# OChicken/GPQHE

Hardware: AMD Instinct MI355X
Metric: ciphertext he_mul/sec (RNS core: tensor 30 limbs + key-switch 45 limbs), N=2^16 (higher is better)
Workload: dtype u64; 1 GPU; he_mul RNS core, n=2^16, dimA=30, dimB=45, batch=64 ciphertexts per GPU (BASELINE configs[2]); he_rescale has no RNS-domain work in the reference; batch_per_gpu=64, total_batch=64, chunk=32, parallelism=ciphertext-per-GPU x1, no data-path collective, launcher=single process

## Files before the change

gpqhe_amd/_native.py:

```python
import ctypes as C
import os

_HERE = os.path.dirname(os.path.abspath(__file__))
LIB_PATH = os.path.join(_HERE, "libgpqhe_hip.so")


def use_variant(path):
    global LIB_PATH
    if _lib is not None:
        raise RuntimeError("use_variant(%r): the library is already loaded" % path)
    if not os.path.exists(path):
        raise FileNotFoundError(path)
    LIB_PATH = os.path.abspath(path)


u64 = C.c_uint64
vp = C.c_void_p

SIGNATURES = {
    "gpq_ctx_create": (C.c_int, [C.POINTER(vp), C.c_uint, C.c_uint, C.c_int]),
    "gpq_ctx_create_from_tables": (C.c_int, [C.POINTER(vp), C.c_uint, C.c_uint, C.POINTER(u64),
                                             C.POINTER(C.POINTER(u64)), C.POINTER(C.POINTER(u64)), C.c_int]),
    "gpq_ctx_destroy": (None, [vp]),
    "gpq_ctx_logn": (C.c_uint, [vp]),
# ... 28 lines not shown
    "gpq_mulpt_rns": (C.c_int, [vp] * 6 + [C.c_uint, C.c_uint, vp]),
    "gpq_set_chunk": (C.c_int, [vp, C.c_uint]),
    "gpq_set_limb_block": (C.c_int, [vp, C.c_uint]),
    "gpq_set_limb_classes": (C.c_int, [vp, C.c_uint, C.c_uint]),
    "gpq_tensor_workspace_bytes": (C.c_size_t, [vp, C.c_uint, C.c_uint]),
    "gpq_keyswitch_workspace_bytes": (C.c_size_t, [vp, C.c_uint, C.c_uint]),
    "gpq_he_mul_tensor": (C.c_int, [vp] * 8 + [C.c_uint, C.c_uint, vp, vp]),
    "gpq_keyswitch": (C.c_int, [vp] * 6 + [C.c_uint, C.c_uint, vp, vp]),
    "gpq_big_words": (C.c_uint, [C.c_uint]),
    "gpq_ctx_phat_invmp": (u64, [vp, C.c_uint, C.c_uint]),
    "gpq_ctx_pbits": (C.c_uint, [vp, C.c_uint]),
    "gpq_rns_decompose": (C.c_int, [vp, vp, vp, C.c_uint, C.c_uint, C.c_uint, vp]),
    "gpq_rns_decompose_limbs": (C.c_int, [vp, vp, vp, C.c_uint, C.c_uint, C.c_uint, C.c_uint, vp]),
    "gpq_rns_reconstruct": (C.c_int, [vp, vp, C.c_uint, vp, C.c_uint, C.c_uint, C.c_uint, vp]),
    "gpq_rns_reconstruct_one": (C.c_int, [vp, C.POINTER(u64), C.c_uint, C.POINTER(u64), C.c_uint]),
    "gpq_set_exact_crt": (C.c_int, [vp, C.c_int]),
    "gpq_set_stream_bridge": (C.c_int, [vp, C.c_int]),
    "gpq_debug_force_redo": (C.c_int, [vp, C.c_uint]),
    "gpq_debug_split_entry_fits_wide": (C.c_int, [u64, u64, u64]),
    "gpq_debug_zero_watch": (C.c_int, [vp, C.c_int]),
    "gpq_debug_zero_flags": (C.c_long, [vp, vp, vp, C.c_size_t]),
    "gpq_set_lazy_decompose": (C.c_int, [vp, C.c_int]),
    "gpq_set_nt_policy": (C.c_int, [vp, C.c_int]),
    "gpq_set_overlap": (C.c_int, [vp, C.c_int]),
    "gpq_last_lanes": (C.c_uint, [vp]),
    "gpq_debug_fail_peer": (C.c_int, [vp, C.c_int]),
    "gpq_debug_table_bytes": (C.c_size_t, [vp, C.c_int]),
    "gpq_set_fused_tail": (C.c_int, [vp, C.c_int]),
    "gpq_big_transpose": (C.c_int, [vp, vp, vp, C.c_uint, C.c_uint, C.c_int, vp]),
    "gpq_big_addsub": (C.c_int, [vp, vp, vp, vp, C.c_uint, C.c_uint, C.c_int, vp]),
    "gpq_set_prescale": (C.c_int, [vp, C.c_int]),
    "gpq_set_bridge_mfma": (C.c_int, [vp, C.c_int]),
    "gpq_poly_mul_workspace_bytes": (C.c_size_t, [vp, C.c_uint, C.c_uint]),
    "gpq_poly_mul": (C.c_int, [vp, vp, vp, vp, C.c_uint, C.c_uint, C.c_uint, C.c_uint, vp, vp]),
    "gpq_poly_mul_general_workspace_bytes": (C.c_size_t, [vp, C.c_uint, C.c_uint]),
    "gpq_rns_reconstruct_general": (C.c_int, [vp, vp, C.c_uint, vp, C.c_uint, C.c_uint, C.POINTER(u64), C.c_uint, vp, vp]),
    "gpq_poly_mul_general": (C.c_int, [vp, vp, vp, vp, C.c_uint, C.c_uint, C.POINTER(u64), C.c_uint, C.c_uint, vp, vp]),
    "gpq_he_rs": (C.c_int, [vp, vp, vp, C.c_uint, C.c_uint, C.c_uint, C.c_uint, vp]),
    "gpq_he_rescale": (C.c_int, [vp, vp, vp, C.c_uint, C.c_uint, C.c_uint, C.c_uint, vp]),
    "gpq_he_dims": (C.c_int, [vp, C.c_uint, C.c_uint] + [C.POINTER(C.c_uint)] * 4),
    "gpq_he_mul_workspace_bytes": (C.c_size_t, [vp, C.c_uint, C.c_uint, C.c_uint, C.c_uint, C.c_uint]),
    "gpq_he_mul": (C.c_int, [vp] * 9 + [C.c_uint] * 6 + [vp, vp]),
    "gpq_he_mul_rs": (C.c_int, [vp] * 9 + [C.c_uint] * 7 + [vp, vp]),
    "gpq_relin_tail_workspace_bytes": (C.c_size_t, [vp, C.c_uint, C.c_uint, C.c_uint, C.c_uint]),
    "gpq_relin_tail": (C.c_int, [vp, vp, vp, vp, C.c_uint, C.c_uint, C.c_uint, C.c_uint, C.c_uint, vp, vp]),
    "gpq_relin_tail_overwriting": (C.c_int, [vp, vp, vp, vp, C.c_uint, C.c_uint, C.c_uint, C.c_uint, C.c_uint, vp, vp]),
# ... 133 lines not shown
```

gpqhe_amd/csrc/engine.hip:

```cpp
#include "../../include/gpqhe_hip.h"
#include "engine_internal.hpp"
#include "ntt_kernels.hpp"

#include <cmath>
#include <cstdlib>
#include <cstdarg>
#include <cstdio>
#include <cstring>
#include <new>
#include <type_traits>

using namespace gpq;

static thread_local char g_err[512] = "";

int gpq_fail(int code, const char *fmt, ...) {
  va_list ap;
  va_start(ap, fmt);
  vsnprintf(g_err, sizeof g_err, fmt, ap);
  va_end(ap);
  return code;
}
extern "C" const char *gpq_last_error(void) { return g_err; }

// ... 417 lines not shown
template <typename TW_, int LOW_, bool NT_>
struct Mid8Inst { using TW = TW_; static constexpr int LOW = LOW_; static constexpr bool NT = NT_; };
template <typename F>
static int launch_mid8(const gpq_ctx *c, const PassArgs &m, unsigned limbs, const uint64_t **evk0, const uint64_t **evk1, int slot, hipStream_t s, F launch) {
  return for_limb_ranges<true>(c, m, limbs, evk0, evk1, [&](auto tag, const PassArgs &a, unsigned nl) {
    using TW = decltype(tag);
    ProfScope prof(c, slot, s);
    with_nt(a.nt, [&](auto nt) {
      constexpr bool NT = decltype(nt)::value;
      if (c->low9) launch(Mid8Inst<TW, 9, NT>{}, a, nl);
      else launch(Mid8Inst<TW, 8, NT>{}, a, nl);
    });
    return (int)GPQ_OK;
  });
}
template <typename K>
static int launch_mid8(const gpq_ctx *c, const PassArgs &m, unsigned limbs, unsigned polys, int slot, hipStream_t s, K kernel) {
  return launch_mid8(c, m, limbs, nullptr, nullptr, slot, s, [&](auto inst, const PassArgs &a, unsigned nl) {
    hipLaunchKernelGGL(kernel(inst), dim3(c->n >> 11, polys, nl), dim3(CONTIG_WAVES * 64), 0, s, a);
  });
}
template <typename K, typename... Tail>
static int launch_keyswitch_mid8(const gpq_ctx *c, KeyswitchArgs m, unsigned limbs, unsigned polys, int slot, hipStream_t s, K kernel, Tail... tail) {
  return launch_mid8(c, m.p, limbs, &m.evk0, &m.evk1, slot, s, [&](auto inst, const PassArgs &a, unsigned nl) {
    KeyswitchArgs ka{a, m.evk0, m.evk1};
    const dim3 block(CONTIG_WAVES * 64);
    if (polys / 2) hipLaunchKernelGGL(kernel(inst, std::true_type{}), dim3(c->n >> 11, polys / 2, nl), block, 0, s, ka, 0u, tail...);
    if (polys & 1) hipLaunchKernelGGL(kernel(inst, std::false_type{}), dim3(c->n >> 11, 1, nl), block, 0, s, ka, polys - 1, tail...);
  });
}

template <int M1, int EL, bool INV, bool CANON, typename TW, int CW = 8>
int launch_strided_t(const PassArgs &a, unsigned gy, unsigned gz, hipStream_t s) {
  using G = StridedGeom<M1, EL>;
  with_nt(a.nt, [&](auto nt) {
    hipLaunchKernelGGL((strided_pass<M1, EL, INV, CANON, TW, CW, decltype(nt)::value>), dim3((1u << CW) >> G::CB, gy, gz), dim3(G::T), 0, s, a);
  });
  return GPQ_OK;
}

template <bool INV>
int launch_strided(const gpq_ctx *c, const PassArgs &args, unsigned dim, unsigned polys, hipStream_t s) {
  return for_limb_ranges<true>(c, args, dim, nullptr, nullptr, [&](auto tag, const PassArgs &a, unsigned limbs) {
    using TW = decltype(tag);
    ProfScope prof(c, INV ? GPQ_K_STRIDED_INV : GPQ_K_STRIDED_FWD, s);
    switch (c->logn) {
      case 13: return launch_strided_t<5, 4, INV, false, TW>(a, polys * a.nslab, limbs, s);
      case 14: return launch_strided_t<6, 4, INV, false, TW>(a, polys * a.nslab, limbs, s);
// ... 314 lines not shown
      for (unsigned i = 0; i < nin; ++i) m.src[i] = f.dst[i];
      m.dst[0] = d0 + k0 * poly + loff; m.dst[1] = d1 + k0 * poly + loff; m.dst[2] = d2 + k0 * poly + loff;
      if ((rc = launch_mid8(c, m, limbs, polys, GPQ_K_TENSOR_MID, s, [&](auto i) {
            using I = decltype(i);
            return square ? tensor_sq_mid8<typename I::TW, I::LOW, I::NT> : tensor_mid8<typename I::TW, I::LOW, I::NT>;
          }))) return rc;
      PassArgs b = make_args(c, dim, 3, nt);
      b.limb0 = l0;
      if (inv_tabs) b.tabs = inv_tabs;
      for (int i = 0; i < 3; ++i) { b.src[i] = m.dst[i]; b.dst[i] = m.dst[i]; }
      if ((rc = launch_strided<true>(c, b, limbs, polys, s))) return rc;
    }
    return (int)GPQ_OK;
  };
  if ((rc = gpq_launch_groups(c, s, batch, chunk, gpq_lane_key(3, dim, chunk, 0, 0, 0), [&](gpq_ctx *q) { return inv_tabs ? 0 : gpq_tensor_workspace_bytes(q, dim, chunk); }, own, peer))) return rc;
  return after_launch("gpq_he_mul_tensor");
}

extern "C" int gpq_keyswitch(gpq_ctx *c, uint64_t *c0, uint64_t *c1, const uint64_t *x,
                             const uint64_t *evk0, const uint64_t *evk1,
                             unsigned dim, unsigned batch, void *workspace, void *stream) {
  return gpq_keyswitch_scaled(c, c0, c1, x, evk0, evk1, dim, batch, workspace, stream, nullptr);
}
int gpq_keyswitch_scaled(gpq_ctx *c, uint64_t *c0, uint64_t *c1, const uint64_t *x, const uint64_t *evk0, const uint64_t *evk1, unsigned dim,
                         unsigned batch, void *workspace, void *stream, const LimbTab *inv_tabs) {
  int rc = check_shape(c, dim, batch, "gpq_keyswitch");
  if (rc) return rc;
  if (!c0 || !c1 || !x || !evk0 || !evk1 || !workspace) return gpq_fail(GPQ_ERR_INVALID, "gpq_keyswitch: null pointer");
  hipStream_t s = (hipStream_t)stream;
  const size_t poly = (size_t)dim << c->logn;
  uint64_t *ws = (uint64_t *)workspace;

  if (!two_pass(c)) {
    HIP_TRY(hipMemcpyAsync(ws, x, batch * poly * 8, hipMemcpyDeviceToDevice, s));
    if ((rc = gpq_ntt(c, ws, dim, batch, stream))) return rc;
    for (unsigned k = 0; k < batch; ++k) {
      if ((rc = gpq_rns_mul(c, c0 + k * poly, ws + k * poly, evk0, dim, 1, stream))) return rc;
      if ((rc = gpq_rns_mul(c, c1 + k * poly, ws + k * poly, evk1, dim, 1, stream))) return rc;
    }
    if ((rc = gpq_invntt(c, c0, dim, batch, stream))) return rc;
    return gpq_invntt(c, c1, dim, batch, stream);
  }

  const unsigned chunk = gpq_group_size(c, batch);
  const unsigned lblock = limb_block(c, dim);
  auto peer = [&](const PeerLane &lane, unsigned k0, unsigned polys) {
    const size_t o = k0 * poly;
    return gpq_keyswitch_scaled(lane.c, c0 + o, c1 + o, x + o, evk0, evk1, dim, polys, lane.ws, lane.s, inv_tabs);
  };
  auto own = [&](unsigned k0, unsigned polys) {
    int rc;
    for (unsigned l0 = 0; l0 < dim; l0 += lblock) {
      const unsigned limbs = dim - l0 < lblock ? dim - l0 : lblock;
      const size_t loff = (size_t)l0 << c->logn;
      StageRange stage("gpq_keyswitch: strided fwd / keyswitch_mid8x2 / strided inv x2");
      const unsigned nt = nt_for(c, polys, limbs, 3);
      PassArgs f = make_args(c, dim, 1, nt);
      f.limb0 = l0;
      f.src[0] = x + k0 * poly + loff; f.dst[0] = ws + loff;
      if ((rc = launch_strided<false>(c, f, limbs, polys, s))) return rc;
      KeyswitchArgs m;
      m.p = make_args(c, dim, 1, nt);
      m.p.limb0 = l0;
      m.p.src[0] = f.dst[0]; m.p.dst[0] = c0 + k0 * poly + loff; m.p.dst[1] = c1 + k0 * poly + loff;
      m.evk0 = evk0 + loff; m.evk1 = evk1 + loff;
      if ((rc = launch_keyswitch_mid8(c, m, limbs, polys, GPQ_K_KEYSWITCH_MID, s, [](auto i, auto two) {
            using I = decltype(i);
            return keyswitch_mid8x2<typename I::TW, I::LOW, decltype(two)::value, I::NT>;
          }))) return rc;
      PassArgs b = make_args(c, dim, 2, nt);
      b.limb0 = l0;
      if (inv_tabs) b.tabs = inv_tabs;
      for (int i = 0; i < 2; ++i) { b.src[i] = m.p.dst[i]; b.dst[i] = m.p.dst[i]; }
      if ((rc = launch_strided<true>(c, b, limbs, polys, s))) return rc;
    }
    return (int)GPQ_OK;
  };
  if ((rc = gpq_launch_groups(c, s, batch, chunk, gpq_lane_key(4, dim, chunk, 0, 0, 0), [&](gpq_ctx *q) { return inv_tabs ? 0 : gpq_keyswitch_workspace_bytes(q, dim, chunk); }, own, peer))) return rc;
  return after_launch("gpq_keyswitch");
}

extern "C" int gpq_automorphism_index(unsigned logn, uint64_t g, uint32_t *idx) {
  if (logn < 1 || logn > 17 || !(g & 1) || !idx) return gpq_fail(GPQ_ERR_INVALID, "gpq_automorphism_index: logn in [1, 17], odd g, idx");
  const uint64_t n = 1ull << logn, m = 2 * n, gm = g & (m - 1);
  auto brv = [logn](uint64_t x) { uint64_t r = 0; for (unsigned b = 0; b < logn; ++b) r |= ((x >> b) & 1) << (logn - 1 - b); return r; };
  for (uint64_t j = 0; j < n; ++j) idx[j] = (uint32_t)brv((((2 * brv(j) + 1) * gm) & (m - 1)) >> 1);
  return GPQ_OK;
}

int gpq_hoist_forward(gpq_ctx *c, uint64_t *slab, unsigned dim, unsigned polys, hipStream_t s) {
  PassArgs a = make_args(c, dim, 1, nt_for(c, polys, dim, 1));
  a.src[0] = a.dst[0] = slab;
  int rc;
  if (!two_pass(c)) {
    for (unsigned k0 = 0; k0 < polys; k0 += kMaxPolysPerLaunch) {
      const unsigned cnt = polys - k0 < kMaxPolysPerLaunch ? polys - k0 : kMaxPolysPerLaunch;
      a.src[0] = a.dst[0] = slab + (size_t)k0 * ((size_t)dim << c->logn);
      if ((rc = launch_small<false>(c, a, dim, cnt, s))) return rc;
    }
    return after_launch("gpq_he_rot_hoisted: forward transform");
  }
  if ((rc = launch_strided<false>(c, a, dim, polys, s))) return rc;
// ... 4 lines not shown
int gpq_keyswitch_rotated(gpq_ctx *c, uint64_t *c0, uint64_t *c1, const uint64_t *X, const uint64_t *evk0, const uint64_t *evk1,
                          unsigned dim, unsigned polys, unsigned g, void *workspace, hipStream_t s, const LimbTab *inv_tabs) {
  const size_t poly = (size_t)dim << c->logn;
  int rc;
  if (!two_pass(c)) {
    uint64_t *ws = (uint64_t *)workspace;
    const size_t rows = (size_t)polys * dim;
    for (size_t r0 = 0; r0 < rows; r0 += 65535) {
      const unsigned cnt = rows - r0 < 65535 ? (unsigned)(rows - r0) : 65535u;
      ProfScope prof(c, GPQ_K_AUTOMORPHISM_GATHER, s);
      hipLaunchKernelGGL(automorphism_gather, dim3((c->n + 255) / 256, cnt), dim3(256), 0, s, X + (r0 << c->logn), ws + (r0 << c->logn), c->logn, g);
    }
    for (unsigned k = 0; k < polys; ++k) {
      if ((rc = gpq_rns_mul(c, c0 + k * poly, ws + k * poly, evk0, dim, 1, s))) return rc;
      if ((rc = gpq_rns_mul(c, c1 + k * poly, ws + k * poly, evk1, dim, 1, s))) return rc;
    }
    if ((rc = gpq_invntt(c, c0, dim, polys, s))) return rc;
    return gpq_invntt(c, c1, dim, polys, s);
  }
  const unsigned nt = nt_for(c, polys, dim, 3);
  KeyswitchArgs m;
  m.p = make_args(c, dim, 1, nt);
  m.p.src[0] = X; m.p.dst[0] = c0; m.p.dst[1] = c1;
  m.evk0 = evk0; m.evk1 = evk1;
  if ((rc = launch_keyswitch_mid8(c, m, dim, polys, GPQ_K_KEYSWITCH_ROT_MID, s, [](auto i, auto two) {
        using I = decltype(i);
        return keyswitch_rot_mid8x2<typename I::TW, I::LOW, decltype(two)::value, I::NT>;
      }, g))) return rc;
  PassArgs b = make_args(c, dim, 2, nt);
  if (inv_tabs) b.tabs = inv_tabs;
  b.src[0] = b.dst[0] = c0; b.src[1] = b.dst[1] = c1;
  if ((rc = launch_strided<true>(c, b, dim, polys, s))) return rc;
  return after_launch("gpq_he_rot_hoisted: key switch");
}

int gpq_gemv_mac(gpq_ctx *c, uint64_t *acc0, uint64_t *acc1, const uint64_t *r0, const uint64_t *r1, const uint64_t *diag,
                 const void *terms, unsigned nterms, unsigned dim, unsigned polys, hipStream_t s) {
  constexpr int BT = 4;
  GemvMacArgs a{c->d_tabs, r0, r1, diag, acc0, acc1, (const uint2 *)terms, nterms, polys, dim, c->logn};
  const dim3 grid((polys + BT - 1) / BT, c->n >= 512 ? c->n / 512 : 1, dim);
  ProfScope prof(c, GPQ_K_GEMV_MAC, s);
  with_nt(nt_for(c, (size_t)polys * (nterms ? nterms : 1), dim, 2), [&](auto nt) {
    hipLaunchKernelGGL((gemv_mac<BT, decltype(nt)::value>), grid, dim3(256), 0, s, a);
  });
  return after_launch("gemv_mac");
}

extern "C" int gpq_set_nt_policy(gpq_ctx *c, int mode) {
  if (!c) return gpq_fail(GPQ_ERR_INVALID, "gpq_set_nt_policy: null context");
  if (mode < -1 || mode > 1) return gpq_fail(GPQ_ERR_INVALID, "gpq_set_nt_policy: mode %d (want -1 by working set, 0 never, 1 always)", mode);
  c->set.nt_mode = mode;
  return GPQ_OK;
}

extern "C" int gpq_set_limb_classes(gpq_ctx *c, unsigned wide, unsigned split) {
  if (!c) return gpq_fail(GPQ_ERR_INVALID, "gpq_set_limb_classes: null context");
  c->set.nsplit = split < c->nsplit_tables ? split : c->nsplit_tables;
  c->set.nwide = wide < c->nwide_max ? wide : c->nwide_max;
  if (c->set.nwide > c->set.nsplit) c->set.nwide = c->set.nsplit;
  return GPQ_OK;
}

extern "C" int gpq_debug_split_entry_fits_wide(uint64_t p, uint64_t x, uint64_t y) {
  if (p <= (1ull << 59) || p - (1ull << 59) >= GPQ_WIDE_CMAX || x > p || y > p) return -1;
  return split_entry_fits_wide(p, x, y) ? 1 : 0;
}

extern "C" int gpq_set_limb_block(gpq_ctx *c, unsigned limbs) {
  if (!c) return gpq_fail(GPQ_ERR_INVALID, "gpq_set_limb_block: null context");
  c->set.limb_block = limbs;
  return GPQ_OK;
}

extern "C" int gpq_set_chunk(gpq_ctx *c, unsigned chunk) {
  if (!c || chunk < 1 || chunk > kMaxPolysPerLaunch) return gpq_fail(GPQ_ERR_INVALID, "gpq_set_chunk: bad arguments");
  c->set.chunk = chunk;
// ... 99 lines not shown
```

gpqhe_amd/csrc/engine_internal.hpp:

```cpp
#pragma once
#include <atomic>
#include <cstdio>
#include <map>
#include <memory>
#include <set>
#include <string>
#include <utility>
#include <vector>
#include "tables.hpp"

struct gpq_ctx;
int gpq_fail(int code, const char *fmt, ...);

inline bool gpq_capturing(hipStream_t s, bool *query_failed = nullptr) {
  hipStreamCaptureStatus cap = hipStreamCaptureStatusNone;
  const bool ok = hipStreamIsCapturing(s, &cap) == hipSuccess;
  if (query_failed) *query_failed = !ok;
  return ok && cap != hipStreamCaptureStatusNone;
}

template <typename T>
struct gpq_dev {
  T *p = nullptr;
  size_t bytes = 0;
// ... 80 lines not shown
  gpq_dev<void> d_bfrag_w;
  gpq_dev<uint64_t> d_pk_w, d_tkp_w;
  gpq_dev<gpq::LimbTab> d_tabs_w;
  bool direct_tried = false;
  gpq_recon_mfma direct;
  std::map<unsigned, gpq_recon_mfma> direct_padded;
  const gpq::LimbTab *d_tabs_direct = nullptr;
  gpq_dev<uint64_t> d_scale, d_unscale;
};

struct gpq_table_cache {
  size_t device_bytes = 0;
  gpq_dev<uint64_t> d_w, d_winv;
  gpq_dev<gpq::TwS> d_ws, d_winvs;
  gpq_dev<gpq::LimbTab> d_tabs;
  std::vector<gpq::LimbTab> h_tabs;
  std::map<std::pair<unsigned, unsigned>, gpq_bridge_basis> bases;
  std::map<std::pair<unsigned, unsigned>, gpq_relin_tables> relins;
  std::map<std::pair<std::pair<unsigned, unsigned>, unsigned>, gpq_decomp_mfma> decomps;
  gpq_dev<uint16_t> d_error_table;
  std::map<const gpq::LimbTab *, unsigned> scaled_wide_limit;
};

struct gpq_settings {
  unsigned chunk = 32;
  unsigned limb_block = 0;
  unsigned nsplit = 0;
  unsigned nwide = 0;
  bool bridge_mfma = true;
  bool lazy_decompose = true;
  unsigned debug_force_redo = 0;
  int nt_mode = -1;
  bool stream_bridge = true;
  bool exact_crt = false;
  bool prescale = true;
  bool prescale_upper = true;
  bool tail_direct = true;
  bool fuse_tail = false;
};

struct gpq_ctx {
  int device = 0;
  unsigned logn = 0, n = 0, nprimes = 0;
  gpq_settings set;
  std::vector<uint64_t> p, pinv_mont, pinv_barr, ninv_mont, psi;
  std::vector<uint64_t> zetas, zetas_inv;
  std::shared_ptr<gpq_table_cache> cache;
  bool tables_borrowed = false;
  const uint64_t *d_w = nullptr, *d_winv = nullptr;
  const gpq::TwS *d_ws = nullptr, *d_winvs = nullptr;
  const gpq::LimbTab *d_tabs = nullptr;
  unsigned nsplit_tables = 0;
  bool low9 = false;
  unsigned nwide_max = 0;
  gpq_dev<unsigned char> d_redo;
  std::vector<gpq_dev<void>> retired;
  gpq_dev<unsigned> d_wave_any;
  int overlap = -1;
  bool peer_failed = false;
  size_t peer_ws_declined = 0;
  int debug_peer_fail = 0;
  unsigned last_lanes = 1;
  std::set<unsigned long long> peer_warm;
  gpq_ctx *peer = nullptr;
  gpq_stream_own peer_stream;
  gpq_event ev_fork, ev_join;
  gpq_dev<void> peer_ws;
  gpq_dev<unsigned> d_zflag;
  gpq_dev<unsigned> d_zwatch;
  size_t zwatch_cap = 0, zwatch_count = 0;
  bool prof_on = false;
  std::vector<gpq_prof_rec> prof;
  std::vector<gpq_event> prof_pool;
};

struct DeviceScope {
  int prev = -1;
  explicit DeviceScope(int device) { if (hipGetDevice(&prev) != hipSuccess) prev = -1; (void)hipSetDevice(device); }
  ~DeviceScope() { if (prev >= 0) (void)hipSetDevice(prev); }
};

template <typename T>
template <typename U>
int gpq_dev<T>::upload(gpq_ctx *c, const std::vector<U> &v) {
  DeviceScope on_device(c->device);
  hipError_t e = alloc(v.size() * sizeof(U));
  if (e == hipSuccess) {
    counted = &c->cache->device_bytes; *counted += bytes;
    e = hipMemcpy(p, v.data(), bytes, hipMemcpyHostToDevice);
  }
// ... 164 lines not shown
```

gpqhe_amd/csrc/ntt_kernels.hpp:

```cpp
#pragma once
#include "modarith.hpp"
#include "tables.hpp"

namespace gpq {

template <bool NT> __device__ __forceinline__ uint64_t slab_ld(const uint64_t *p) {
  if constexpr (NT) return __builtin_nontemporal_load(p);
  else return *p;
}
template <bool NT> __device__ __forceinline__ void slab_st(uint64_t *p, uint64_t v) {
  if constexpr (NT) __builtin_nontemporal_store(v, p);
  else *p = v;
}


constexpr int tw_count(int EL, int BHI, int BLO) { return (1 << (EL - BLO)) - (1 << (EL - BHI - 1)); }

constexpr int tw_off(int EL, int BHI, int b) { return (1 << (EL - b - 1)) - (1 << (EL - BHI - 1)); }

template <int EL, int BHI, int B, int BLO, bool UNIFORM, int NTW, typename TW>
__device__ __forceinline__ void load_tw_bits(TW (&tw)[NTW], unsigned ibase, int rs, unsigned logn,
                                             const TW *__restrict__ w) {
  const int sh = rs + B + 1;
  const TW *wp = w + (1u << (logn - sh)) + (UNIFORM ? 0u : (ibase >> sh));
#pragma unroll
// ... 360 lines not shown
          zero_note(a, zm, p0 + j, blockIdx.z);
          store_h<NT>(dst + (size_t)j * a.poly_stride, x[j], ln);
        }
    } else {
      tw.load_l(ln, wave0, a.logn, wt);
#pragma unroll
      for (int j = 0; j < CONTIG_POLYS; ++j)
        if (j < (int)cnt) {
          ln.h_to_l(x[j]);
          gs_group<4, 3, 0, true>(x[j], tw.t, k);
          ln.l_to_h(x[j]);
        }
      tw.load_h(ln, wave0, a.logn, wt);
#pragma unroll
      for (int j = 0; j < CONTIG_POLYS; ++j)
        if (j < (int)cnt) {
          gs_group<4, 3, 0>(x[j], tw.t, k);
          store_h<NT>(dst + (size_t)j * a.poly_stride, x[j], ln);
        }
    }
  }
}

struct KeyswitchArgs { PassArgs p; const uint64_t *evk0; const uint64_t *evk1; };

constexpr int LANE8_LDS_PER_WAVE = 576;

template <int LOW>
struct Lane8 {
  static constexpr int JB = LOW - 3;
  static constexpr int MB = LOW - 6;
  static constexpr int LHI = LOW - 7;
  unsigned hk, mk, lk;
  uint64_t *lds;
  __device__ __forceinline__ Lane8(uint64_t *wave_lds) {
    const unsigned lane = threadIdx.x & 63, j = lane & ((1u << JB) - 1), blk = lane >> JB;
    hk = (blk << LOW) + j;
    mk = (blk << LOW) + ((j >> MB) << JB) + (j & ((1u << MB) - 1));
    lk = (blk << LOW) + (j << 3);
    lds = wave_lds;
  }
  __device__ static __forceinline__ unsigned pad1(unsigned l) { return l + ((l >> JB) << MB); }
  __device__ static __forceinline__ unsigned pad2(unsigned l) { return l + (l >> 3); }
  __device__ __forceinline__ void h_to_m(uint64_t (&x)[8]) const {
#pragma unroll
    for (int e = 0; e < 8; ++e) lds[pad1(hk + (e << JB))] = x[e];
    wave_lds_sync();
// ... 201 lines not shown
  using TT = TwTraits<TW>;
  __shared__ uint64_t lds[CONTIG_WAVES * LANE8_LDS_PER_WAVE];
  uint64_t m[8], x[8], y[8];
  Mid8<TW, LOW, NT> s(lds, a);
  const size_t off = s.off(a, blockIdx.y);
  const PrimeK &k = s.k;
  s.load_first(m, a.src[0] + off);
  s.load(x, a.src[1] + off);
  s.load(y, a.src[2] + off);
  s.forward(m, x, y);
  s.load_inverse_l();
#pragma unroll
  for (int e = 0; e < 8; ++e) {
    const uint64_t u = TT::left(m[e], k);
    x[e] = TT::inv_from4(mulmod_lazy(u, TT::right(x[e], k), k), k);
    y[e] = TT::inv_from4(mulmod_lazy(u, TT::right(y[e], k), k), k);
  }
  s.inverse(x, y);
  s.finish(x); s.ln.store_h(a.dst[0] + off, x);
  s.finish(y); s.ln.store_h(a.dst[1] + off, y);
}

#define GPQ_KEYSWITCH_PRODUCTS()                                  \
  s.ln.load_l(e0, ka.evk0 + koff);                                \
  s.ln.load_l(e1, ka.evk1 + koff);                                \
  s.load_inverse_l();                                             \
  uint64_t y0[8], y1[8];                                          \
  _Pragma("unroll") for (int e = 0; e < 8; ++e) {                 \
    const uint64_t u0 = TT::right(x0[e], k);                      \
    x0[e] = TT::inv_from4(mulmod_lazy(u0, e0[e], k), k);          \
    y0[e] = TT::inv_from4(mulmod_lazy(u0, e1[e], k), k);          \
  }                                                               \
  if constexpr (TWO) {                                            \
    _Pragma("unroll") for (int e = 0; e < 8; ++e) {               \
      const uint64_t u1 = TT::right(x1[e], k);                    \
      x1[e] = TT::inv_from4(mulmod_lazy(u1, e0[e], k), k);        \
      y1[e] = TT::inv_from4(mulmod_lazy(u1, e1[e], k), k);        \
    }                                                             \
  }
template <bool TWO, typename S>
__device__ __forceinline__ void keyswitch_back(S &s, const PassArgs &a, uint64_t (&x0)[8], uint64_t (&y0)[8], uint64_t (&x1)[8], uint64_t (&y1)[8], size_t off0, size_t off1) {
  if constexpr (TWO) s.inverse(x0, y0, x1, y1);
  else s.inverse(x0, y0);
  s.finish(x0); s.ln.store_h(a.dst[0] + off0, x0);
  s.finish(y0); s.ln.store_h(a.dst[1] + off0, y0);
  if constexpr (TWO) {
    s.finish(x1); s.ln.store_h(a.dst[0] + off1, x1);
    s.finish(y1); s.ln.store_h(a.dst[1] + off1, y1);
  }
}

template <typename TW, int LOW, bool TWO = true, bool NT = false>
__global__ __launch_bounds__(CONTIG_WAVES * 64, TWO ? 4 : 3) void keyswitch_mid8x2(KeyswitchArgs ka, unsigned first) {
  using TT = TwTraits<TW>;
  __shared__ uint64_t lds[CONTIG_WAVES * LANE8_LDS_PER_WAVE];
  const PassArgs &a = ka.p;
  Mid8<TW, LOW, NT> s(lds, a);
  const unsigned wave0 = s.wave0;
  const PrimeK &k = s.k;
  const unsigned p0 = first + 2 * blockIdx.y;
  const size_t off0 = s.off(a, p0);
  const size_t off1 = TWO ? off0 + a.poly_stride : off0;
  const size_t koff = ((size_t)blockIdx.z << a.logn) + wave0;
  uint64_t x0[8], x1[8], e0[8], e1[8];
  s.load_first(x0, a.src[0] + off0);
  if constexpr (TWO) { s.load(x1, a.src[0] + off1); s.forward(x0, x1); }
  else s.forward(x0);
  GPQ_KEYSWITCH_PRODUCTS();
  keyswitch_back<TWO>(s, a, x0, y0, x1, y1, off0, off1);
}

__device__ __forceinline__ unsigned automorphism_src(unsigned j, unsigned logn, unsigned g) {
  const unsigned mask2n = (2u << logn) - 1;
  const unsigned e = (((__brev(j) >> (32 - logn)) << 1) | 1u) * g & mask2n;
  return __brev(e >> 1) >> (32 - logn);
}

template <typename TW, int LOW, bool TWO = true, bool NT = false>
__global__ __launch_bounds__(CONTIG_WAVES * 64, TWO ? 4 : 3) void keyswitch_rot_mid8x2(KeyswitchArgs ka, unsigned first, unsigned g) {
  using TT = TwTraits<TW>;
  using L8 = Lane8N<LOW, NT>;
  __shared__ uint64_t lds[CONTIG_WAVES * LANE8_LDS_PER_WAVE];
  const PassArgs &a = ka.p;
  Mid8<TW, LOW, NT> s(lds, a);
  const unsigned wave0 = s.wave0;
  const PrimeK &k = s.k;
  const unsigned p0 = first + 2 * blockIdx.y;
  const size_t off0 = (size_t)p0 * a.poly_stride + ((size_t)blockIdx.z << a.logn) + wave0;
  const size_t off1 = TWO ? off0 + a.poly_stride : off0;
  const size_t koff = ((size_t)blockIdx.z << a.logn) + wave0;
  const L8 &ln = s.ln;
  const unsigned src0 = automorphism_src(wave0, a.logn, g) & ~511u;
  const size_t soff0 = off0 - wave0 + src0, soff1 = off1 - wave0 + src0;
  unsigned sl[8];
#pragma unroll
  for (int e = 0; e < 8; ++e) sl[e] = automorphism_src(wave0 + ln.lk + e, a.logn, g) & 511u;
  auto gather = [&](uint64_t (&x)[8], size_t soff) {
    ln.load_h(x, a.src[0] + soff);
#pragma unroll
    for (int e = 0; e < 8; ++e) ln.lds[L8::pad2(ln.hk + (e << L8::JB))] = x[e];
    wave_lds_sync();
#pragma unroll
    for (int e = 0; e < 8; ++e) x[e] = ln.lds[L8::pad2(sl[e])];
    wave_lds_sync();
  };
  uint64_t x0[8], x1[8], e0[8], e1[8];
  gather(x0, soff0);
  if constexpr (TWO) gather(x1, soff1);
  GPQ_KEYSWITCH_PRODUCTS();
  keyswitch_back<TWO>(s, a, x0, y0, x1, y1, off0, off1);
}
#undef GPQ_KEYSWITCH_PRODUCTS

__global__ __launch_bounds__(256) void automorphism_gather(const uint64_t *__restrict__ src, uint64_t *__restrict__ dst, unsigned logn, unsigned g) {
  const unsigned j = blockIdx.x * 256 + threadIdx.x;
  if (j >= (1u << logn)) return;
  const size_t row = (size_t)blockIdx.y << logn;
  dst[row + j] = src[row + automorphism_src(j, logn, g)];
}

typedef unsigned long long v2u64 __attribute__((ext_vector_type(2)));
struct GemvMacArgs {
  const LimbTab *tabs;
  const uint64_t *r0, *r1;
  const uint64_t *diag;
  uint64_t *acc0, *acc1;
  const uint2 *terms;
  unsigned nterms, polys, dim, logn;
};
// ... 222 lines not shown
```

gpqhe_amd/engine.py:

```python
import ctypes as C

import numpy as np

from . import _native


def _torch():
    import torch
    return torch


def _ptr(t):
    return C.c_void_p(t.data_ptr())


def _stream():
    torch = _torch()
    return C.c_void_p(torch.cuda.current_stream().cuda_stream)


def to_device(a, device=None):
    torch = _torch()
    a = np.ascontiguousarray(a, dtype=np.uint64)
    return torch.from_numpy(a.view(np.int64)).to(device or "cuda")
# ... 77 lines not shown
        _native.check(self.lib.gpq_set_prescale(self.h, mode), "gpq_set_prescale")

    def set_stream_bridge(self, on):
        _native.check(self.lib.gpq_set_stream_bridge(self.h, 1 if on else 0), "gpq_set_stream_bridge")

    def set_lazy_decompose(self, on):
        _native.check(self.lib.gpq_set_lazy_decompose(self.h, 1 if on else 0), "gpq_set_lazy_decompose")

    def set_overlap(self, on):
        v = -1 if (on is not True and on is not False and int(on) < 0) else (1 if on else 0)
        _native.check(self.lib.gpq_set_overlap(self.h, v), "gpq_set_overlap")

    def debug_fail_peer(self, on=True):
        _native.check(self.lib.gpq_debug_fail_peer(self.h, int(on)), "gpq_debug_fail_peer")

    def debug_table_bytes(self, which=0):
        return int(self.lib.gpq_debug_table_bytes(self.h, which))

    def last_lanes(self):
        return int(self.lib.gpq_last_lanes(self.h))

    def set_nt_policy(self, mode):
        _native.check(self.lib.gpq_set_nt_policy(self.h, int(mode)), "gpq_set_nt_policy")

    def debug_force_redo(self, every):
        _native.check(self.lib.gpq_debug_force_redo(self.h, int(every)), "gpq_debug_force_redo")

    def debug_zero_watch(self, on=True):
        _native.check(self.lib.gpq_debug_zero_watch(self.h, 1 if on else 0), "gpq_debug_zero_watch")

    def debug_zero_flags(self, count):
        before, after = np.zeros(count, dtype=np.uint32), np.zeros(count, dtype=np.uint32)
        got = self.lib.gpq_debug_zero_flags(self.h, before.ctypes.data_as(C.c_void_p), after.ctypes.data_as(C.c_void_p), count)
        if got != count:
            raise RuntimeError("gpq_debug_zero_flags: %d words watched, %d asked for" % (got, count))
        return before, after

    def set_exact_crt(self, on):
        _native.check(self.lib.gpq_set_exact_crt(self.h, 1 if on else 0), "gpq_set_exact_crt")

    def poly_mul(self, r, a, b, W, dim, logq):
        torch = _torch()
        batch = a.numel() // (W * self.n)
        ws = torch.empty(self.lib.gpq_poly_mul_workspace_bytes(self.h, dim, batch) // 8, dtype=torch.int64, device=self._dev)
        _native.check(self.lib.gpq_poly_mul(self.h, self._ptr(r), self._ptr(a), self._ptr(b), W, dim, logq, batch, self._ptr(ws), self._stream()), "gpq_poly_mul")
        return r
# ... 514 lines not shown
```

include/gpqhe_hip.h:

```cpp
#ifndef GPQHE_HIP_H
#define GPQHE_HIP_H

#include <stddef.h>
#include <stdint.h>

#ifdef __cplusplus
extern "C" {
#endif

#define GPQ_OK 0
#define GPQ_ERR_INVALID (-1)
#define GPQ_ERR_HIP (-2)
#define GPQ_ERR_UNSUPPORTED (-3)
#define GPQ_ERR_NOMEM (-4)

typedef struct gpq_ctx gpq_ctx;

int gpq_ctx_create(gpq_ctx **out, unsigned logn, unsigned nprimes, int device);

int gpq_ctx_create_from_tables(gpq_ctx **out, unsigned logn, unsigned nprimes, const uint64_t *primes,
                               const uint64_t *const *zetas_mont, const uint64_t *const *zetas_inv_mont, int device);
void gpq_ctx_destroy(gpq_ctx *ctx);

unsigned gpq_ctx_logn(const gpq_ctx *ctx);
// ... 48 lines not shown

int gpq_keyswitch(gpq_ctx *ctx, uint64_t *c0, uint64_t *c1, const uint64_t *x,
                  const uint64_t *evk0, const uint64_t *evk1,
                  unsigned dim, unsigned batch, void *workspace, void *stream);

unsigned gpq_big_words(unsigned bits);
uint64_t gpq_ctx_phat_invmp(gpq_ctx *ctx, unsigned dim, unsigned d);
unsigned gpq_ctx_pbits(gpq_ctx *ctx, unsigned dim);

int gpq_rns_decompose(gpq_ctx *ctx, uint64_t *slab, const uint64_t *big, unsigned W, unsigned dim, unsigned batch, void *stream);
int gpq_rns_decompose_limbs(gpq_ctx *ctx, uint64_t *slab, const uint64_t *big, unsigned W, unsigned first, unsigned count,
                            unsigned batch, void *stream);
int gpq_rns_reconstruct_one(gpq_ctx *ctx, uint64_t *words, unsigned Wout, const uint64_t *residues, unsigned dim);
int gpq_rns_reconstruct(gpq_ctx *ctx, uint64_t *big, unsigned Wout, const uint64_t *slab, unsigned dim, unsigned batch,
                        unsigned logq, void *stream);
int gpq_set_exact_crt(gpq_ctx *ctx, int on);
int gpq_set_stream_bridge(gpq_ctx *ctx, int on);
int gpq_set_overlap(gpq_ctx *ctx, int on);
unsigned gpq_last_lanes(const gpq_ctx *ctx);
int gpq_debug_fail_peer(gpq_ctx *ctx, int on);
size_t gpq_debug_table_bytes(const gpq_ctx *ctx, int which);
int gpq_set_lazy_decompose(gpq_ctx *ctx, int on);
int gpq_set_nt_policy(gpq_ctx *ctx, int mode);
int gpq_debug_force_redo(gpq_ctx *ctx, unsigned every);
int gpq_debug_split_entry_fits_wide(uint64_t p, uint64_t x, uint64_t y);
int gpq_debug_zero_watch(gpq_ctx *ctx, int on);
long gpq_debug_zero_flags(gpq_ctx *ctx, unsigned *before, unsigned *after, size_t capacity);
int gpq_set_fused_tail(gpq_ctx *ctx, int on);
int gpq_set_prescale(gpq_ctx *ctx, int on);
int gpq_set_bridge_mfma(gpq_ctx *ctx, int on);

size_t gpq_poly_mul_workspace_bytes(const gpq_ctx *ctx, unsigned dim, unsigned batch);
int gpq_poly_mul(gpq_ctx *ctx, uint64_t *r, const uint64_t *a, const uint64_t *b, unsigned W, unsigned dim, unsigned logq,
                 unsigned batch, void *workspace, void *stream);
size_t gpq_poly_mul_general_workspace_bytes(gpq_ctx *ctx, unsigned dim, unsigned batch);
int gpq_rns_reconstruct_general(gpq_ctx *ctx, uint64_t *big, unsigned Wout, const uint64_t *slab, unsigned dim, unsigned batch,
                                const uint64_t *q_words, unsigned Lq, void *scratch, void *stream);
int gpq_poly_mul_general(gpq_ctx *ctx, uint64_t *r, const uint64_t *a, const uint64_t *b, unsigned W, unsigned dim,
                         const uint64_t *q_words, unsigned Lq, unsigned batch, void *workspace, void *stream);

int gpq_he_rs(gpq_ctx *ctx, uint64_t *c0, uint64_t *c1, unsigned W, unsigned logDelta, unsigned logql, unsigned batch, void *stream);
int gpq_he_rescale(gpq_ctx *ctx, uint64_t *c0, uint64_t *c1, unsigned W, unsigned logDelta, unsigned logql, unsigned batch, void *stream);

int gpq_he_dims(gpq_ctx *ctx, unsigned logqL, unsigned logql, unsigned *dimP, unsigned *dimA, unsigned *dimB, unsigned *dimevk);

size_t gpq_he_mul_workspace_bytes(gpq_ctx *ctx, unsigned W, unsigned dimA, unsigned dimB, unsigned dimP, unsigned batch);
// ... 120 lines not shown
```

Before: 7763 he_mul/s.

## Precompute evaluation keys in split Shoup form for keyswitch pointwise products

Adds a per-call pre-pass (evk_split) that converts the evaluation keys for the split-class limbs into a Shoup-like split form (negated value plus precomputed quotient). The keyswitch mid kernel then multiplies with mulmod_split instead of a lazy Montgomery multiply and inverse conversion. It also drops the TT::right/inv_from4 steps and software-pipelines the key loads. This is meant to cut modular-multiply ALU work in the keyswitch inner step. In exchange it adds an extra kernel per call that reads both keys and writes twice-as-wide key data, which raises memory traffic. It is enabled by default for batch of at least 32.

Measured after the change: 7754 he_mul/s. About the same (-0.1%).

```diff
diff --git a/gpqhe_amd/_native.py b/gpqhe_amd/_native.py
--- a/gpqhe_amd/_native.py
+++ b/gpqhe_amd/_native.py
@@ -74,6 +74,8 @@
     "gpq_debug_zero_flags": (C.c_long, [vp, vp, vp, C.c_size_t]),
     "gpq_set_lazy_decompose": (C.c_int, [vp, C.c_int]),
     "gpq_set_nt_policy": (C.c_int, [vp, C.c_int]),
+    "gpq_set_split_keys": (C.c_int, [vp, C.c_int]),
+    "gpq_last_key_form": (C.c_int, [vp]),
     "gpq_set_overlap": (C.c_int, [vp, C.c_int]),
     "gpq_last_lanes": (C.c_uint, [vp]),
     "gpq_debug_fail_peer": (C.c_int, [vp, C.c_int]),
diff --git a/gpqhe_amd/csrc/engine.hip b/gpqhe_amd/csrc/engine.hip
--- a/gpqhe_amd/csrc/engine.hip
+++ b/gpqhe_amd/csrc/engine.hip
@@ -463,8 +463,10 @@
 }
 template <typename K, typename... Tail>
 static int launch_keyswitch_mid8(const gpq_ctx *c, KeyswitchArgs m, unsigned limbs, unsigned polys, int slot, hipStream_t s, K kernel, Tail... tail) {
+  const unsigned limb0 = m.p.limb0;
   return launch_mid8(c, m.p, limbs, &m.evk0, &m.evk1, slot, s, [&](auto inst, const PassArgs &a, unsigned nl) {
-    KeyswitchArgs ka{a, m.evk0, m.evk1};
+    const size_t done = (size_t)(a.limb0 - limb0) << c->logn;
+    KeyswitchArgs ka{a, m.evk0, m.evk1, m.evs0 ? m.evs0 + done : nullptr, m.evs1 ? m.evs1 + done : nullptr};
     const dim3 block(CONTIG_WAVES * 64);
     if (polys / 2) hipLaunchKernelGGL(kernel(inst, std::true_type{}), dim3(c->n >> 11, polys / 2, nl), block, 0, s, ka, 0u, tail...);
     if (polys & 1) hipLaunchKernelGGL(kernel(inst, std::false_type{}), dim3(c->n >> 11, 1, nl), block, 0, s, ka, polys - 1, tail...);
@@ -825,31 +827,39 @@
                              unsigned dim, unsigned batch, void *workspace, void *stream) {
   return gpq_keyswitch_scaled(c, c0, c1, x, evk0, evk1, dim, batch, workspace, stream, nullptr);
 }
-int gpq_keyswitch_scaled(gpq_ctx *c, uint64_t *c0, uint64_t *c1, const uint64_t *x, const uint64_t *evk0, const uint64_t *evk1, unsigned dim,
-                         unsigned batch, void *workspace, void *stream, const LimbTab *inv_tabs) {
-  int rc = check_shape(c, dim, batch, "gpq_keyswitch");
-  if (rc) return rc;
-  if (!c0 || !c1 || !x || !evk0 || !evk1 || !workspace) return gpq_fail(GPQ_ERR_INVALID, "gpq_keyswitch: null pointer");
-  hipStream_t s = (hipStream_t)stream;
+constexpr unsigned kSplitKeysMinBatch = 32;
+struct SplitKeys { const TwS *k0 = nullptr, *k1 = nullptr; };
+static int split_keys(gpq_ctx *c, const uint64_t *evk0, const uint64_t *evk1, unsigned dim, unsigned batch, hipStream_t s, SplitKeys *out) {
+  const int mode = c->set.split_keys;
+  const unsigned limbs = dim < c->set.nsplit ? dim : c->set.nsplit;
+  c->last_key_form = 0;
+  if (!limbs || mode == 0 || (mode < 0 && batch < kSplitKeysMinBatch)) return GPQ_OK;
+  const size_t words = (size_t)limbs << c->logn, need = (size_t)2 * ((size_t)dim << c->logn) * sizeof(TwS);
+  if (need > c->d_evs.bytes) {
+    if (mode < 0 && gpq_capturing(s)) return GPQ_OK;
+    if (int rc = c->d_evs.grow(c, s, need, false, "the first gpq_keyswitch with split-form keys at a new size allocates their slabs: run it once outside stream capture")) return rc;
+  }
+  TwS *o0 = c->d_evs, *o1 = o0 + words;
+  EvkSplitArgs a{c->d_tabs, {evk0, evk1}, {o0, o1}, c->logn, 0};
+  {
+    ProfScope prof(c, GPQ_K_POINTWISE, s);
+    hipLaunchKernelGGL(evk_split, dim3(c->n >> 11, limbs, 2), dim3(CONTIG_WAVES * 64), 0, s, a);
+  }
+  out->k0 = o0; out->k1 = o1;
+  c->last_key_form = 1;
+  return after_launch("evk_split");
+}
+
+static int keyswitch_groups(gpq_ctx *c, uint64_t *c0, uint64_t *c1, const uint64_t *x, const uint64_t *evk0, const uint64_t *evk1, SplitKeys sk, unsigned dim,
+                            unsigned batch, void *workspace, hipStream_t s, const LimbTab *inv_tabs) {
+  int rc;
   const size_t poly = (size_t)dim << c->logn;
   uint64_t *ws = (uint64_t *)workspace;
-
-  if (!two_pass(c)) {
-    HIP_TRY(hipMemcpyAsync(ws, x, batch * poly * 8, hipMemcpyDeviceToDevice, s));
-    if ((rc = gpq_ntt(c, ws, dim, batch, stream))) return rc;
-    for (unsigned k = 0; k < batch; ++k) {
-      if ((rc = gpq_rns_mul(c, c0 + k * poly, ws + k * poly, evk0, dim, 1, stream))) return rc;
-      if ((rc = gpq_rns_mul(c, c1 + k * poly, ws + k * poly, evk1, dim, 1, stream))) return rc;
-    }
-    if ((rc = gpq_invntt(c, c0, dim, batch, stream))) return rc;
-    return gpq_invntt(c, c1, dim, batch, stream);
-  }
-
   const unsigned chunk = gpq_group_size(c, batch);
   const unsigned lblock = limb_block(c, dim);
   auto peer = [&](const PeerLane &lane, unsigned k0, unsigned polys) {
     const size_t o = k0 * poly;
-    return gpq_keyswitch_scaled(lane.c, c0 + o, c1 + o, x + o, evk0, evk1, dim, polys, lane.ws, lane.s, inv_tabs);
+    return keyswitch_groups(lane.c, c0 + o, c1 + o, x + o, evk0, evk1, sk, dim, polys, lane.ws, lane.s, inv_tabs);
   };
   auto own = [&](unsigned k0, unsigned polys) {
     int rc;
@@ -867,9 +877,14 @@
       m.p.limb0 = l0;
       m.p.src[0] = f.dst[0]; m.p.dst[0] = c0 + k0 * poly + loff; m.p.dst[1] = c1 + k0 * poly + loff;
       m.evk0 = evk0 + loff; m.evk1 = evk1 + loff;
-      if ((rc = launch_keyswitch_mid8(c, m, limbs, polys, GPQ_K_KEYSWITCH_MID, s, [](auto i, auto two) {
+      m.evs0 = sk.k0 ? sk.k0 + loff : nullptr; m.evs1 = sk.k1 ? sk.k1 + loff : nullptr;
+      const bool split = sk.k0 != nullptr;
+      if ((rc = launch_keyswitch_mid8(c, m, limbs, polys, GPQ_K_KEYSWITCH_MID, s, [split](auto i, auto two) {
             using I = decltype(i);
-            return keyswitch_mid8x2<typename I::TW, I::LOW, decltype(two)::value, I::NT>;
+            constexpr bool TWO = decltype(two)::value;
+            if constexpr (!std::is_same<typename I::TW, uint64_t>::value)
+              if (split) return keyswitch_mid8x2<typename I::TW, I::LOW, TWO, I::NT, true>;
+            return keyswitch_mid8x2<typename I::TW, I::LOW, TWO, I::NT, false>;
           }))) return rc;
       PassArgs b = make_args(c, dim, 2, nt);
       b.limb0 = l0;
@@ -881,6 +896,30 @@
   };
   if ((rc = gpq_launch_groups(c, s, batch, chunk, gpq_lane_key(4, dim, chunk, 0, 0, 0), [&](gpq_ctx *q) { return inv_tabs ? 0 : gpq_keyswitch_workspace_bytes(q, dim, chunk); }, own, peer))) return rc;
   return after_launch("gpq_keyswitch");
+}
+
+int gpq_keyswitch_scaled(gpq_ctx *c, uint64_t *c0, uint64_t *c1, const uint64_t *x, const uint64_t *evk0, const uint64_t *evk1, unsigned dim,
+                         unsigned batch, void *workspace, void *stream, const LimbTab *inv_tabs) {
+  int rc = check_shape(c, dim, batch, "gpq_keyswitch");
+  if (rc) return rc;
+  if (!c0 || !c1 || !x || !evk0 || !evk1 || !workspace) return gpq_fail(GPQ_ERR_INVALID, "gpq_keyswitch: null pointer");
+  hipStream_t s = (hipStream_t)stream;
+  const size_t poly = (size_t)dim << c->logn;
+  uint64_t *ws = (uint64_t *)workspace;
+
+  if (!two_pass(c)) {
+    HIP_TRY(hipMemcpyAsync(ws, x, batch * poly * 8, hipMemcpyDeviceToDevice, s));
+    if ((rc = gpq_ntt(c, ws, dim, batch, stream))) return rc;
+    for (unsigned k = 0; k < batch; ++k) {
+      if ((rc = gpq_rns_mul(c, c0 + k * poly, ws + k * poly, evk0, dim, 1, stream))) return rc;
+      if ((rc = gpq_rns_mul(c, c1 + k * poly, ws + k * poly, evk1, dim, 1, stream))) return rc;
+    }
+    if ((rc = gpq_invntt(c, c0, dim, batch, stream))) return rc;
+    return gpq_invntt(c, c1, dim, batch, stream);
+  }
+  SplitKeys sk;
+  if ((rc = split_keys(c, evk0, evk1, dim, batch, s, &sk))) return rc;
+  return keyswitch_groups(c, c0, c1, x, evk0, evk1, sk, dim, batch, workspace, s, inv_tabs);
 }
 
 extern "C" int gpq_automorphism_index(unsigned logn, uint64_t g, uint32_t *idx) {
@@ -931,7 +970,7 @@
   KeyswitchArgs m;
   m.p = make_args(c, dim, 1, nt);
   m.p.src[0] = X; m.p.dst[0] = c0; m.p.dst[1] = c1;
-  m.evk0 = evk0; m.evk1 = evk1;
+  m.evk0 = evk0; m.evk1 = evk1; m.evs0 = m.evs1 = nullptr;
   if ((rc = launch_keyswitch_mid8(c, m, dim, polys, GPQ_K_KEYSWITCH_ROT_MID, s, [](auto i, auto two) {
         using I = decltype(i);
         return keyswitch_rot_mid8x2<typename I::TW, I::LOW, decltype(two)::value, I::NT>;
@@ -961,6 +1000,14 @@
   c->set.nt_mode = mode;
   return GPQ_OK;
 }
+
+extern "C" int gpq_set_split_keys(gpq_ctx *c, int mode) {
+  if (!c) return gpq_fail(GPQ_ERR_INVALID, "gpq_set_split_keys: null context");
+  if (mode < -1 || mode > 1) return gpq_fail(GPQ_ERR_INVALID, "gpq_set_split_keys: mode %d (want -1 by batch size, 0 never, 1 always)", mode);
+  c->set.split_keys = mode;
+  return GPQ_OK;
+}
+extern "C" int gpq_last_key_form(const gpq_ctx *c) { return c ? c->last_key_form : -1; }
 
 extern "C" int gpq_set_limb_classes(gpq_ctx *c, unsigned wide, unsigned split) {
   if (!c) return gpq_fail(GPQ_ERR_INVALID, "gpq_set_limb_classes: null context");
diff --git a/gpqhe_amd/csrc/engine_internal.hpp b/gpqhe_amd/csrc/engine_internal.hpp
--- a/gpqhe_amd/csrc/engine_internal.hpp
+++ b/gpqhe_amd/csrc/engine_internal.hpp
@@ -126,6 +126,9 @@
   std::map<const gpq::LimbTab *, unsigned> scaled_wide_limit;
 };
 
+#ifndef GPQ_SPLIT_KEYS_DEFAULT
+#define GPQ_SPLIT_KEYS_DEFAULT -1
+#endif
 struct gpq_settings {
   unsigned chunk = 32;
   unsigned limb_block = 0;
@@ -135,6 +138,7 @@
   bool lazy_decompose = true;
   unsigned debug_force_redo = 0;
   int nt_mode = -1;
+  int split_keys = GPQ_SPLIT_KEYS_DEFAULT;
   bool stream_bridge = true;
   bool exact_crt = false;
   bool prescale = true;
@@ -170,6 +174,8 @@
   gpq_stream_own peer_stream;
   gpq_event ev_fork, ev_join;
   gpq_dev<void> peer_ws;
+  gpq_dev<gpq::TwS> d_evs;
+  int last_key_form = 0;
   gpq_dev<unsigned> d_zflag;
   gpq_dev<unsigned> d_zwatch;
   size_t zwatch_cap = 0, zwatch_count = 0;
diff --git a/gpqhe_amd/csrc/ntt_kernels.hpp b/gpqhe_amd/csrc/ntt_kernels.hpp
--- a/gpqhe_amd/csrc/ntt_kernels.hpp
+++ b/gpqhe_amd/csrc/ntt_kernels.hpp
@@ -1,6 +1,7 @@
 #pragma once
 #include "modarith.hpp"
 #include "tables.hpp"
+#include <type_traits>
 
 namespace gpq {
 
@@ -407,7 +408,25 @@
   }
 }
 
-struct KeyswitchArgs { PassArgs p; const uint64_t *evk0; const uint64_t *evk1; };
+struct KeyswitchArgs { PassArgs p; const uint64_t *evk0; const uint64_t *evk1; const TwS *evs0; const TwS *evs1; };
+
+struct EvkSplitArgs { const LimbTab *tabs; const uint64_t *evk[2]; TwS *out[2]; unsigned logn, limb0; };
+__global__ __launch_bounds__(CONTIG_WAVES * 64) void evk_split(EvkSplitArgs a) {
+  const unsigned lane = threadIdx.x & 63, tile = blockIdx.x * CONTIG_WAVES + (threadIdx.x >> 6);
+  if (tile >= (1u << a.logn) >> 9) return;
+  const PrimeK k = a.tabs[a.limb0 + blockIdx.y].k;
+  const size_t base = ((size_t)blockIdx.y << a.logn) + ((size_t)tile << 9);
+  const ulonglong2 *__restrict__ src = reinterpret_cast<const ulonglong2 *>(a.evk[blockIdx.z] + base + 8 * lane);
+  TwS *__restrict__ dst = a.out[blockIdx.z] + base + lane;
+  uint64_t w[8];
+#pragma unroll
+  for (int i = 0; i < 4; ++i) { const ulonglong2 t = src[i]; w[2 * i] = t.x; w[2 * i + 1] = t.y; }
+#pragma unroll
+  for (int e = 0; e < 8; ++e) {
+    const uint64_t r = csub1(w[e], k);
+    dst[64 * e] = TwS{k.p - r, k.p - mulmod_canon(r, 1ull << 31, k)};
+  }
+}
 
 constexpr int LANE8_LDS_PER_WAVE = 576;
 
@@ -655,20 +674,40 @@
 }
 
 #define GPQ_KEYSWITCH_PRODUCTS()                                  \
-  s.ln.load_l(e0, ka.evk0 + koff);                                \
-  s.ln.load_l(e1, ka.evk1 + koff);                                \
-  s.load_inverse_l();                                             \
   uint64_t y0[8], y1[8];                                          \
-  _Pragma("unroll") for (int e = 0; e < 8; ++e) {                 \
-    const uint64_t u0 = TT::right(x0[e], k);                      \
-    x0[e] = TT::inv_from4(mulmod_lazy(u0, e0[e], k), k);          \
-    y0[e] = TT::inv_from4(mulmod_lazy(u0, e1[e], k), k);          \
-  }                                                               \
-  if constexpr (TWO) {                                            \
+  if constexpr (SK) {                                             \
+    const TwS *__restrict__ q0 = ka.evs0 + koff + (threadIdx.x & 63), *__restrict__ q1 = ka.evs1 + koff + (threadIdx.x & 63); \
+    s.load_inverse_l();                                           \
+    TwS k0 = q0[0], k1 = q1[0];                                   \
     _Pragma("unroll") for (int e = 0; e < 8; ++e) {               \
-      const uint64_t u1 = TT::right(x1[e], k);                    \
-      x1[e] = TT::inv_from4(mulmod_lazy(u1, e0[e], k), k);        \
-      y1[e] = TT::inv_from4(mulmod_lazy(u1, e1[e], k), k);        \
+      const TwS n0 = q0[64 * (e < 7 ? e + 1 : e)], n1 = q1[64 * (e < 7 ? e + 1 : e)]; \
+      const uint64_t u0 = x0[e];                                  \
+      x0[e] = mulmod_split(u0, k0, k);                            \
+      y0[e] = mulmod_split(u0, k1, k);                            \
+      if constexpr (TWO) {                                        \
+        const uint64_t u1 = x1[e];                                \
+        x1[e] = mulmod_split(u1, k0, k);                          \
+        y1[e] = mulmod_split(u1, k1, k);                          \
+      }                                                           \
+      __builtin_amdgcn_sched_barrier(0);                          \
+      k0 = n0; k1 = n1;                                           \
+    }                                                             \
+  } else {                                                        \
+    uint64_t e0[8], e1[8];                                        \
+    s.ln.load_l(e0, ka.evk0 + koff);                              \
+    s.ln.load_l(e1, ka.evk1 + koff);                              \
+    s.load_inverse_l();                                           \
+    _Pragma("unroll") for (int e = 0; e < 8; ++e) {               \
+      const uint64_t u0 = TT::right(x0[e], k);                    \
+      x0[e] = TT::inv_from4(mulmod_lazy(u0, e0[e], k), k);        \
+      y0[e] = TT::inv_from4(mulmod_lazy(u0, e1[e], k), k);        \
+    }                                                             \
+    if constexpr (TWO) {                                          \
+      _Pragma("unroll") for (int e = 0; e < 8; ++e) {             \
+        const uint64_t u1 = TT::right(x1[e], k);                  \
+        x1[e] = TT::inv_from4(mulmod_lazy(u1, e0[e], k), k);      \
+        y1[e] = TT::inv_from4(mulmod_lazy(u1, e1[e], k), k);      \
+      }                                                           \
     }                                                             \
   }
 template <bool TWO, typename S>
@@ -683,8 +722,9 @@
   }
 }
 
-template <typename TW, int LOW, bool TWO = true, bool NT = false>
+template <typename TW, int LOW, bool TWO = true, bool NT = false, bool SK = false>
 __global__ __launch_bounds__(CONTIG_WAVES * 64, TWO ? 4 : 3) void keyswitch_mid8x2(KeyswitchArgs ka, unsigned first) {
+  static_assert(!SK || !std::is_same<TW, uint64_t>::value, "split-form keys: split and wide limbs only");
   using TT = TwTraits<TW>;
   __shared__ uint64_t lds[CONTIG_WAVES * LANE8_LDS_PER_WAVE];
   const PassArgs &a = ka.p;
@@ -695,7 +735,7 @@
   const size_t off0 = s.off(a, p0);
   const size_t off1 = TWO ? off0 + a.poly_stride : off0;
   const size_t koff = ((size_t)blockIdx.z << a.logn) + wave0;
-  uint64_t x0[8], x1[8], e0[8], e1[8];
+  uint64_t x0[8], x1[8];
   s.load_first(x0, a.src[0] + off0);
   if constexpr (TWO) { s.load(x1, a.src[0] + off1); s.forward(x0, x1); }
   else s.forward(x0);
@@ -737,7 +777,8 @@
     for (int e = 0; e < 8; ++e) x[e] = ln.lds[L8::pad2(sl[e])];
     wave_lds_sync();
   };
-  uint64_t x0[8], x1[8], e0[8], e1[8];
+  uint64_t x0[8], x1[8];
+  constexpr bool SK = false;
   gather(x0, soff0);
   if constexpr (TWO) gather(x1, soff1);
   GPQ_KEYSWITCH_PRODUCTS();
diff --git a/gpqhe_amd/engine.py b/gpqhe_amd/engine.py
--- a/gpqhe_amd/engine.py
+++ b/gpqhe_amd/engine.py
@@ -123,6 +123,12 @@
 
     def set_nt_policy(self, mode):
         _native.check(self.lib.gpq_set_nt_policy(self.h, int(mode)), "gpq_set_nt_policy")
+
+    def set_split_keys(self, mode):
+        _native.check(self.lib.gpq_set_split_keys(self.h, int(mode)), "gpq_set_split_keys")
+
+    def last_key_form(self):
+        return int(self.lib.gpq_last_key_form(self.h))
 
     def debug_force_redo(self, every):
         _native.check(self.lib.gpq_debug_force_redo(self.h, int(every)), "gpq_debug_force_redo")
diff --git a/include/gpqhe_hip.h b/include/gpqhe_hip.h
--- a/include/gpqhe_hip.h
+++ b/include/gpqhe_hip.h
@@ -94,6 +94,8 @@
 size_t gpq_debug_table_bytes(const gpq_ctx *ctx, int which);
 int gpq_set_lazy_decompose(gpq_ctx *ctx, int on);
 int gpq_set_nt_policy(gpq_ctx *ctx, int mode);
+int gpq_set_split_keys(gpq_ctx *ctx, int mode);
+int gpq_last_key_form(const gpq_ctx *ctx);
 int gpq_debug_force_redo(gpq_ctx *ctx, unsigned every);
 int gpq_debug_split_entry_fits_wide(uint64_t p, uint64_t x, uint64_t y);
 int gpq_debug_zero_watch(gpq_ctx *ctx, int on);
```
